# IvanTyulyandin/HMM_FASTA_Viterbi

Hardware: AMD Instinct MI355X
Metric: M residues/sec (GCUPS) for profile M=1400 vs 100k seqs, 1/2/4/8 GPU (higher is better)
Workload: dtype f32

## Files before the change

### hmm_fasta_viterbi_amd/_native.py

```python
from __future__ import annotations

import ctypes as C
import os

LIB_DIR = os.path.join(os.path.dirname(os.path.abspath(__file__)), "lib")
LIB_PATH = os.environ.get("MSV_LIB_PATH") or os.path.join(LIB_DIR, "libmsv_hip.so")

STATUS = {
    0: "MSV_OK",
    1: "MSV_ERR_INVALID_ARGUMENT",
    2: "MSV_ERR_IO",
    3: "MSV_ERR_PARSE",
    4: "MSV_ERR_BAD_RESIDUE",
    5: "MSV_ERR_SEQUENCE_TOO_LONG",
    6: "MSV_ERR_UNSUPPORTED_MODEL",
    7: "MSV_ERR_NO_DEVICE",
    8: "MSV_ERR_HIP",
    9: "MSV_ERR_OUT_OF_MEMORY",
    10: "MSV_ERR_RCCL",
}
MSV_OK = 0
MSV_ERR_BAD_RESIDUE = 4

EXPORTED = [
    "msv_status_string", "msv_version", "msv_device_count",
    "msv_hmm_read", "msv_hmm_destroy", "msv_hmm_model_length", "msv_hmm_name", "msv_hmm_stats",
    "msv_hmm_match_emissions", "msv_hmm_insert_emissions", "msv_hmm_transitions", "msv_hmm_msv_scores",
    "msv_sequence_transitions",
    "msv_fasta_read", "msv_fasta_destroy", "msv_fasta_count", "msv_fasta_rejected", "msv_fasta_codes",
    "msv_fasta_offsets", "msv_fasta_header", "msv_encode_residues",
    "msv_profile_create", "msv_profile_create_from_hmm", "msv_profile_destroy", "msv_profile_describe",
    "msv_profile_reserve_length", "msv_score_batch", "msv_score_batch_device", "msv_profile_check",
    "msv_order_longest_first", "msv_variant_count", "msv_variant_name", "msv_profile_set_variant",
    "msv_score_grid", "msv_score_grid_device", "msv_pvalues", "msv_pvalues_device",
    "msv_shard_bounds", "msv_score_batch_multi",
    "msv_fasta_parse_device", "msv_fasta_read_device", "msv_fasta_device_destroy", "msv_fasta_device_count",
    "msv_fasta_device_rejected", "msv_fasta_device_residues", "msv_fasta_device_codes", "msv_fasta_device_offsets",
    "msv_fasta_device_header_spans", "msv_fasta_device_text", "msv_fasta_device_download",
    "msv_fasta_device_max_length", "msv_score_fasta_device", "msv_fasta_device_device",
    "msv_score_batch_async", "msv_profile_wait", "msv_profile_bind_stream",
    "msv_multi_create", "msv_multi_score_batch", "msv_multi_destroy",
    "msv_host_alloc", "msv_host_free", "msv_profile_variant_for",
    "msv_filter_select_device", "msv_hmm_viterbi_scores", "msv_vit_cpu_score", "msv_vit_profile_create",
    "msv_vit_profile_create_from_hmm", "msv_vit_profile_destroy", "msv_vit_profile_reserve_length",
    "msv_vit_profile_describe", "msv_vit_variant_count", "msv_vit_variant_name", "msv_vit_profile_set_variant",
    "msv_vit_score_batch_device", "msv_vit_score_batch", "msv_vit_profile_check", "msv_vit_filter_batch",
    "msv_vit_profile_bind_stream",
    "msv_vit_cpu_trace", "msv_vit_trace_plan_count", "msv_vit_trace_plan_name", "msv_vit_trace_plan_capacity",
    "msv_vit_trace_plan_cell", "msv_vit_trace_sequence_bytes", "msv_vit_trace_chunk_cuts", "msv_vit_trace_batch",
    "msv_vit_traces_count", "msv_vit_traces_domains", "msv_vit_traces_ops", "msv_vit_traces_copy",
    "msv_vit_traces_free", "msv_vit_trace_describe", "msv_vit_traces_stats",
    "msv_fwd_cpu_score", "msv_fwd_cpu_score_batch", "msv_fwd_pvalues", "msv_fwd_scan_constants",
    "msv_fwd_profile_create", "msv_fwd_profile_create_from_hmm", "msv_fwd_profile_destroy",
    "msv_fwd_profile_reserve_length", "msv_fwd_profile_describe", "msv_fwd_variant_count", "msv_fwd_variant_name",
    "msv_fwd_profile_set_variant", "msv_fwd_score_batch_device", "msv_fwd_profile_bind_stream",
    "msv_fwd_score_batch", "msv_fwd_profile_check", "msv_fwd_pvalues_device", "msv_fwd_filter_batch",
]


class MSVError(RuntimeError):
    def __init__(self, status: int, what: str = ""):
        self.status = status
        self.name = STATUS.get(status, f"MSV_ERR_{status}")
        super().__init__(f"{what}: {self.name}" if what else self.name)


class KernelInfo(C.Structure):
    _fields_ = [
# ... 147 lines not shown
        "msv_fasta_read": (C.c_int, [C.c_char_p, C.POINTER(vp)]),
        "msv_fasta_destroy": (None, [vp]),
        "msv_fasta_count": (sz, [vp]),
        "msv_fasta_rejected": (sz, [vp]),
        "msv_fasta_codes": (C.POINTER(C.c_uint8), [vp]),
        "msv_fasta_offsets": (C.POINTER(C.c_uint64), [vp]),
        "msv_fasta_header": (C.c_char_p, [vp, sz]),
        "msv_encode_residues": (C.c_int, [C.c_char_p, sz, vp]),
        "msv_profile_create": (C.c_int, [C.c_int, vp, u32, f32, f32, f32, C.POINTER(vp)]),
        "msv_profile_create_from_hmm": (C.c_int, [C.c_int, vp, C.POINTER(vp)]),
        "msv_profile_destroy": (None, [vp]),
        "msv_profile_describe": (C.c_int, [vp, C.POINTER(KernelInfo)]),
        "msv_profile_variant_for": (C.c_char_p, [vp, C.c_uint64]),
        "msv_profile_reserve_length": (C.c_int, [vp, u64]),
        "msv_score_batch": (C.c_int, [vp, vp, vp, u64, vp, vp]),
        "msv_host_alloc": (C.c_int, [sz, C.POINTER(vp)]),
        "msv_host_free": (C.c_int, [vp]),
        "msv_score_batch_device": (C.c_int, [vp, vp, u64, vp, u64, vp, vp, vp]),
        "msv_score_batch_async": (C.c_int, [vp, vp, vp, u64, vp, C.POINTER(C.c_uint64)]),
        "msv_profile_wait": (C.c_int, [vp, u64]),
        "msv_profile_bind_stream": (C.c_int, [vp, vp]),
        "msv_multi_create": (C.c_int, [vp, C.c_uint32, C.POINTER(vp)]),
        "msv_multi_score_batch": (C.c_int, [vp, vp, vp, u64, vp]),
        "msv_multi_destroy": (None, [vp]),
        "msv_profile_check": (C.c_int, [vp, vp]),
        "msv_order_longest_first": (C.c_int, [vp, vp, u64, vp, vp]),
        "msv_variant_count": (C.c_int, []),
        "msv_variant_name": (C.c_char_p, [C.c_int]),
        "msv_profile_set_variant": (C.c_int, [vp, C.c_char_p]),
        "msv_score_grid": (C.c_int, [vp, C.c_uint32, vp, vp, u64, vp, vp]),
        "msv_score_grid_device": (C.c_int, [vp, C.c_uint32, vp, u64, vp, u64, vp, vp, vp]),
        "msv_pvalues": (C.c_int, [vp, vp, u64, C.c_float, C.c_float, vp]),
        "msv_shard_bounds": (C.c_int, [vp, u64, C.c_uint32, vp]),
        "msv_fasta_parse_device": (C.c_int, [C.c_int, vp, u64, vp, vp]),
        "msv_fasta_read_device": (C.c_int, [C.c_int, C.c_char_p, vp, vp]),
        "msv_fasta_device_destroy": (None, [vp]),
        "msv_fasta_device_count": (u64, [vp]),
        "msv_fasta_device_device": (C.c_int, [vp]),
        "msv_fasta_device_rejected": (u64, [vp]),
        "msv_fasta_device_residues": (u64, [vp]),
        "msv_fasta_device_codes": (vp, [vp]),
        "msv_fasta_device_offsets": (vp, [vp]),
        "msv_fasta_device_header_spans": (vp, [vp]),
        "msv_fasta_device_text": (vp, [vp]),
        "msv_fasta_device_download": (C.c_int, [vp, vp, vp, vp]),
        "msv_fasta_device_max_length": (u64, [vp]),
        "msv_score_fasta_device": (C.c_int, [vp, vp, vp]),
        "msv_score_batch_multi": (C.c_int, [vp, C.c_uint32, vp, vp, u64, vp]),
        "msv_pvalues_device": (C.c_int, [C.c_int, vp, vp, u64, C.c_float, C.c_float, vp, vp]),
        "msv_filter_select_device": (C.c_int, [C.c_int, vp, vp, vp, u64, f32, f32, C.c_double, vp, vp, vp, vp]),
        "msv_hmm_viterbi_scores": (C.c_int, [vp, C.c_int, vp, vp, vp, fp, fp, fp]),
        "msv_vit_cpu_score": (C.c_int, [vp, vp, vp, u32, f32, f32, f32, vp, u64, fp]),
        "msv_vit_profile_create": (C.c_int, [C.c_int, vp, vp, vp, u32, f32, f32, f32, C.POINTER(vp)]),
        "msv_vit_profile_create_from_hmm": (C.c_int, [C.c_int, vp, C.c_int, C.POINTER(vp)]),
        "msv_vit_profile_destroy": (None, [vp]),
        "msv_vit_profile_reserve_length": (C.c_int, [vp, u64]),
        "msv_vit_profile_describe": (C.c_int, [vp, C.POINTER(VitInfo)]),
        "msv_vit_variant_count": (C.c_int, []),
        "msv_vit_variant_name": (C.c_char_p, [C.c_int]),
        "msv_vit_profile_set_variant": (C.c_int, [vp, C.c_char_p]),
        "msv_vit_score_batch_device": (C.c_int, [vp, vp, u64, vp, u64, vp, vp, vp, vp]),
        "msv_vit_profile_bind_stream": (C.c_int, [vp, vp]),
        "msv_vit_score_batch": (C.c_int, [vp, vp, vp, u64, vp, vp]),
        "msv_vit_profile_check": (C.c_int, [vp, vp]),
        "msv_vit_filter_batch": (C.c_int, [vp, vp, vp, vp, u64, f32, f32, C.c_double, vp, vp, vp,
                                           C.POINTER(C.c_uint64)]),
# ... 50 lines not shown
```

### hmm_fasta_viterbi_amd/csrc/host_common.cpp

```cpp
#include <algorithm>
#include <cmath>
#include <cstdint>
#include <limits>
#include <vector>

#include "host_cpu.h"
#include "msv.h"
#include "vit_trace_plan.h"

extern "C" {

const char* msv_status_string(msv_status s) {
    switch (s) {
        case MSV_OK: return "MSV_OK";
        case MSV_ERR_INVALID_ARGUMENT: return "MSV_ERR_INVALID_ARGUMENT";
        case MSV_ERR_IO: return "MSV_ERR_IO";
        case MSV_ERR_PARSE: return "MSV_ERR_PARSE";
        case MSV_ERR_BAD_RESIDUE: return "MSV_ERR_BAD_RESIDUE";
        case MSV_ERR_SEQUENCE_TOO_LONG: return "MSV_ERR_SEQUENCE_TOO_LONG";
        case MSV_ERR_UNSUPPORTED_MODEL: return "MSV_ERR_UNSUPPORTED_MODEL";
        case MSV_ERR_NO_DEVICE: return "MSV_ERR_NO_DEVICE";
        case MSV_ERR_HIP: return "MSV_ERR_HIP";
        case MSV_ERR_OUT_OF_MEMORY: return "MSV_ERR_OUT_OF_MEMORY";
        case MSV_ERR_RCCL: return "MSV_ERR_RCCL";
// ... 79 lines not shown
    for (size_t k = 1; k + 1 < model_length; ++k)
        for (int t = 0; t < 7; ++t)
            if (!(transition_scores[k * 7 + t] <= 0.0f)) return MSV_ERR_INVALID_ARGUMENT;
    for (uint64_t i = 0; i < L; ++i)
        if (codes[i] >= 20) return MSV_ERR_BAD_RESIDUE;
    const msv_host::VitTrace t = msv_host::viterbi_trace_on_sequence(
        match_scores, insert_scores, transition_scores, model_length, tr_B_Mk, tr_E_C, tr_E_J, codes, L);
    *score = t.score;
    if (domains) {
        if (*n_domains < t.domains.size() || *n_ops < t.ops.size()) return MSV_ERR_INVALID_ARGUMENT;
        std::copy(t.domains.begin(), t.domains.end(), domains);
        std::copy(t.ops.begin(), t.ops.end(), ops);
    }
    *n_domains = static_cast<uint32_t>(t.domains.size());
    *n_ops = t.ops.size();
    return MSV_OK;
}

msv_status msv_shard_bounds(const uint64_t* offsets, uint64_t n, uint32_t n_shards, uint64_t* bounds) {
    if (!bounds || n_shards == 0 || (n && !offsets)) return MSV_ERR_INVALID_ARGUMENT;
    bounds[0] = 0;
    bounds[n_shards] = n;
    if (n == 0) {
        for (uint32_t k = 1; k < n_shards; ++k) bounds[k] = 0;
        return MSV_OK;
    }
    const uint64_t total = offsets[n] - offsets[0];
    for (uint32_t k = 1; k < n_shards; ++k) {
        const unsigned __int128 q = static_cast<unsigned __int128>(total) * k / n_shards;
        const uint64_t target = offsets[0] + static_cast<uint64_t>(q);
        bounds[k] = static_cast<uint64_t>(std::lower_bound(offsets + 1, offsets + 1 + n, target) - (offsets + 1));
    }
    for (uint32_t k = 1; k <= n_shards; ++k) bounds[k] = std::min(n, std::max(bounds[k], bounds[k - 1]));
    return MSV_OK;
}

}

namespace msv_host {

float run_on_sequence(const float* emission_scores, size_t M, float tr_B_Mk, float tr_E_C, float tr_E_J,
                      const uint8_t* codes, size_t L) {
    constexpr float ninf = -std::numeric_limits<float>::infinity();
    float loop, move;
    msv_sequence_transitions(L, &loop, &move);
    std::vector<float> prev(M, ninf), cur(M, ninf);
    float J = ninf, C = ninf, N = 0.0f, B = move;
    for (size_t i = 0; i < L; ++i) {
        const float* e = emission_scores + static_cast<size_t>(codes[i]) * M;
        const float Bt = B + tr_B_Mk;
        const float* pv = prev.data();
        float* cv = cur.data();
        for (size_t j = 1; j < M; ++j) cv[j] = e[j] + std::max(pv[j - 1], Bt);
        float Ek[8] = {ninf, ninf, ninf, ninf, ninf, ninf, ninf, ninf};
        size_t j = 1;
        for (; j + 8 <= M; j += 8)
            for (int q = 0; q < 8; ++q) Ek[q] = std::max(Ek[q], cv[j + q]);
        for (; j < M; ++j) Ek[0] = std::max(Ek[0], cv[j]);
        float E = ninf;
        for (float x : Ek) E = std::max(E, x);
        J = std::max(J + loop, E + tr_E_J);
        C = std::max(C + loop, E + tr_E_C);
        N = N + loop;
        B = std::max(N + move, J + move);
        std::swap(prev, cur);
    }
// ... 158 lines not shown
```

### hmm_fasta_viterbi_amd/csrc/host_cpu.h

```cpp
#pragma once

#include <cstddef>
#include <cstdint>
#include <vector>

#include "msv.h"

namespace msv_host {

float run_on_sequence(const float* emission_scores, size_t M, float tr_B_Mk, float tr_E_C, float tr_E_J,
                      const uint8_t* codes, size_t L);

float viterbi_run_on_sequence(const float* msc, const float* isc, const float* tsc, size_t M, float tr_B_Mk,
                              float tr_E_C, float tr_E_J, const uint8_t* codes, size_t L);

struct VitTrace {
    float score = 0;
    std::vector<msv_vit_domain> domains;
    std::vector<uint8_t> ops;
};
VitTrace viterbi_trace_on_sequence(const float* msc, const float* isc, const float* tsc, size_t M, float tr_B_Mk,
                                   float tr_E_C, float tr_E_J, const uint8_t* codes, size_t L);

std::vector<float> msv_variant_table(const float* es, uint32_t model_length, int G, int S, int sa);
std::vector<float> msv_coop_table(const float* es, uint32_t model_length, int waves, int S, int sa, int halo);
struct VitTables {
    std::vector<float> et, it, tt;
};
VitTables vit_tables(const float* msc, const float* isc_tab, const float* tsc, uint32_t model_length, int S, int team,
                     bool isc);

}
```

### hmm_fasta_viterbi_amd/csrc/msv_device.cpp

```cpp
#include <hip/hip_runtime.h>

#include <algorithm>
#include <cmath>
#include <cstdio>
#include <cstring>
#include <limits>
#include <map>
#include <memory>
#include <mutex>
#include <new>
#include <thread>
#include <vector>

#include "hip_rt.h"
#include "host_cpu.h"
#include "launch_ring.h"
#include "msv.h"
#include "msv_kernel.h"
#include "msv_plan.h"

using msvplan::CallPlan;
using msvplan::kLaunchSlots;
using msvrt::csr_extent;
using msvrt::CsrStaging;
// ... 122 lines not shown
    streams[device] = st;
    return st;
}

static bool lazy_stream(const msv_profile* p, hipStream_t st) {
    return st == p->stream || st == p->stream2 || (p->bound && st == p->bound) || (p->shared && st == p->shared);
}

static msv_status err_status(uint32_t err) {
    if (err & msvk::kErrBadOrder) return MSV_ERR_INVALID_ARGUMENT;
    if (err & msvk::kErrBadResidue) return MSV_ERR_BAD_RESIDUE;
    if (err & msvk::kErrTooLong) return MSV_ERR_SEQUENCE_TOO_LONG;
    return MSV_OK;
}

static msv_status scan_scores(const float* scores, uint64_t n) {
    bool inf = false, nan = false;
    for (uint64_t i = 0; i < n; ++i) {
        const float x = scores[i];
        inf |= x == std::numeric_limits<float>::infinity();
        nan |= x != x;
    }
    if (inf) return MSV_ERR_BAD_RESIDUE;
    if (nan) return MSV_ERR_SEQUENCE_TOO_LONG;
    return MSV_OK;
}

static msv_status grid_blocks(int device, const void* kernel, int waves, int* blocks) {
    const hipError_t e = msvrt::resident_blocks(device, kernel, waves * 64, blocks);
    return *blocks > 0 ? MSV_OK : hip_status(e);
}

static msv_status install_plan(msv_profile* p, const msvk::Variant* v, Plan& plan) {
    const std::vector<float> tab =
        msv_host::msv_variant_table(p->emission_scores.data(), p->model_length, v->G, v->S, v->sa);
    MSV_HIP(plan.d_etab.replace_with(reinterpret_cast<const float4*>(tab.data()), tab.size() / 4));
    plan.v = v;
    plan.groups_per_block = v->waves * (64 / v->G) * v->streams;
    return grid_blocks(p->device, v->fn, v->waves, &plan.blocks);
}

static void drop_plan(Plan& plan) {
    if (plan.d_etab) (void)hipDeviceSynchronize();
    plan = Plan{};
}

static msv_status install_coop_table(msv_profile* p, const msvk::CoopVariant* cv, Plan& plan) {
    const std::vector<float> tab =
        msv_host::msv_coop_table(p->emission_scores.data(), p->model_length, cv->waves, cv->S, cv->sa, cv->halo);
    MSV_HIP(plan.d_etab.replace_with(reinterpret_cast<const float4*>(tab.data()), tab.size() / 4));
    plan.v = nullptr;
    plan.cv = cv;
    plan.blocks = 0;
    plan.groups_per_block = 1;
    return MSV_OK;
}

static msv_status install_plans(msv_profile* p, int forced) {
    int cus = 0, count = 0;
    MSV_HIP(hipDeviceGetAttribute(&cus, hipDeviceAttributeMultiprocessorCount, p->device));
    const msvk::Variant* all = msvk::variants(&count);
    const msvk::CoopVariant* coop = msvk::coop_variants(&count);
    const auto blocks_of = [&](msvplan::Kind kind, int i) {
        int blocks = 0;
        if (kind == msvplan::kCoop) (void)grid_blocks(p->device, coop[i].fn, coop[i].waves, &blocks);
        else (void)grid_blocks(p->device, all[i].fn, all[i].waves, &blocks);
        return blocks;
    };
// ... 828 lines not shown
```

### hmm_fasta_viterbi_amd/csrc/msv_kernel.h

```cpp
#pragma once

#include <hip/hip_runtime.h>

#include <cstdint>

namespace msvk {

constexpr int kAminoAcids = 20;
constexpr int kPoisonRow = 20;
constexpr int kTableRows = 21;
constexpr int kWideBlocks = 64;
constexpr int kLdsLimit = 163840;

constexpr int kStampWords = 6;
constexpr int kClockTwin = -1;

constexpr uint32_t kErrBadResidue = 1u;
constexpr uint32_t kErrTooLong = 2u;
constexpr uint32_t kErrBadOrder = 4u;
constexpr uint32_t kErrTeamHang = 8u;

constexpr int lds_rows_for(int G, int S) {
    return (kLdsLimit / (G * S * 4)) >= kTableRows ? kTableRows : (kLdsLimit / (G * S * 4));
}

__device__ __host__ inline double msv_pvalue_of(float score, uint64_t L, float mu, float lambda) {
    if (L == 0) return 1.0;
    const float p1 = static_cast<float>(L) / static_cast<float>(L + 1);
    const float nullsc = static_cast<float>(static_cast<double>(L) * log(static_cast<double>(p1)) +
                                            log(1.0 - static_cast<double>(p1)));
    const float bits = (score - nullsc) / 0.69314718055994529f;
    const double y = static_cast<double>(lambda) * (static_cast<double>(bits) - static_cast<double>(mu));
    const double ey = -exp(-y);
    return fabs(ey) < 5e-9 ? -ey : 1.0 - exp(ey);
}

struct KernelArgs {
    const float4* etab;
    const uint8_t* residues;
    const uint64_t* offsets;
    const uint32_t* order;
    const float2* lentab;
    float* scores;
    uint32_t* counter;
    uint32_t* errors;
    uint64_t n;
    uint32_t lentab_n;
    float tr_B_Mk, tr_E_C, tr_E_J;
    uint64_t* stamps;
};

constexpr uint32_t kGridMaxProfiles = 32;
struct GridArgs {
    uint32_t profiles;
    uint32_t per_profile;
    KernelArgs p[kGridMaxProfiles];
// ... 39 lines not shown
```

### hmm_fasta_viterbi_amd/csrc/msv_kernel_body.inc

```
    constexpr bool SPLIT = SA > 0;
    constexpr bool WIDE = RPFO == kWideBlocks;
    constexpr bool CLOCK = RPFO == kClockTwin;
    constexpr int SW = CLOCK ? kStampWords : 4;
    constexpr int RPF0 = (RPFO > 0 && !WIDE) ? RPFO : residue_prefetch<S>();
    using St = Stream<S, (SPLIT && RPF0 < 2) ? 2 : RPF0>;
    static_assert(SPLIT ? (S - SA) % 2 == 0 : S % 4 == 0, "float4 chunks (A block), float2 halves (B block)");
    static_assert(PF >= 1 && D >= 1 && D <= 2, "PF >= 1, D in {1, 2}");
    static_assert(!SPLIT || (G >= 32 && !BIG && D == 1 && SA % 4 == 0 && SA < S), "split: 32/64-lane groups");
    constexpr int C4 = S / 4;
    constexpr int CA = SPLIT ? SA / 4 : C4;
    constexpr int HB = SPLIT ? (S - SA) / 2 : 0;
    constexpr int ROW_F4 = CA * G;
    constexpr int HBP = (HB + 1) & ~1;
    constexpr int LDS_ROWS = SPLIT ? kAminoAcids : lds_rows_for(G, S);
    constexpr bool ROT = !BIG && D == 1 && St::RPF > 1;
    constexpr int BLKN = St::RPF > 1 ? 16 : 0;
    constexpr bool BLK = !BIG && D == 1 && G >= 16 && !SPLIT && BLKN > 0;
    static_assert(!WIDE || BLK, "wide blocks are the zero-copy form of residue blocks");
    constexpr int NPH = BLK ? BLKN : St::RPF;
    constexpr bool XROW = !BIG && !SPLIT && D == 1 && PF >= C4 && St::RPF >= 2;
    constexpr bool XROW2 = XROW && NPH % 2 == 0 && PF <= 2;
    static_assert(SPLIT || BIG == (LDS_ROWS < kTableRows), "BIG <=> table does not fit LDS");
    __shared__ float4 tab[LDS_ROWS * ROW_F4];

    const float NINF = -__builtin_inff();
    const int lane = threadIdx.x & 63;
    const int gl = lane & (G - 1);
    const bool leader = gl == 0;

    for (int i = threadIdx.x; i < LDS_ROWS * ROW_F4; i += WAVES * 64) tab[i] = a.etab[i];
    __syncthreads();

    const uint8_t* __restrict__ res = a.residues;
    const float trBMk = a.tr_B_Mk, tEC = a.tr_E_C, tEJ = a.tr_E_J;
    const bool sameEJ = __float_as_uint(tEC) == __float_as_uint(tEJ);

    uint32_t rows_done = 0;
    constexpr uint32_t kFetchAhead = S >= 64 ? 8 + 256 / S : 0xFFFFFFFFu;
    constexpr uint32_t kNone = 0xFFFFFFFFu;
    const uint32_t n_groups = MSV_BLOCKS * (WAVES * 64 / G);
    static_assert(WAVES % 4 == 0, "waves are dealt in rounds of one per SIMD");
    const uint32_t wave = threadIdx.x >> 6;
    const uint32_t wave_set = a.n <= n_groups ? (wave >> 2) * 4u * MSV_BLOCKS + 4u * MSV_BLOCK + (wave & 3u)
                                              : MSV_BLOCK * WAVES + wave;
    uint32_t pending = wave_set * (64 / G) + static_cast<uint32_t>(lane / G);

    constexpr uint32_t kYoung = S >= 64 ? 8 : 0;
    const bool young = kYoung > 0 && (threadIdx.x >> 6) >= (3u * WAVES) / 4u;
    auto take = [&]() __attribute__((always_inline)) -> uint32_t {
        if constexpr (kYoung > 0) {
            if (young) {
                const uint32_t cur = group_take<G>(a.counter, false, lane, n_groups);
                if (static_cast<uint64_t>(cur) + (static_cast<uint64_t>(n_groups) * kYoung) / 4 >= a.n)
                    return 0xFFFFFFFEu;
            }
        }
        return group_take<G>(a.counter, leader, lane, n_groups);
    };
    using Ph0 = std::integral_constant<int, 0>;
    const uint32_t blk_lane = static_cast<uint32_t>(gl & (BLKN > 0 ? BLKN - 1 : 0));
    std::conditional_t<WIDE, WideBlocks, NoWideBlocks> wb;
    auto load_w = [&](uint32_t a, uint32_t e3, uint32_t& sh) __attribute__((always_inline)) -> uint32_t {
        const uint32_t a2 = min(a, e3);
        uint32_t w;
        __builtin_memcpy(&w, res + a2, 4);
        sh = (a - a2) << 3;
        return w;
    };
    const uint32_t bp_lane = WIDE ? static_cast<uint32_t>(((lane & ~15) + (blk_lane >> 2)) << 2) : 0u;
    const uint32_t bp_shift = WIDE ? (blk_lane & 3u) << 3 : 0u;
    auto extract = [&](uint32_t w, uint32_t k) __attribute__((always_inline)) -> uint32_t {
        const uint32_t v = static_cast<uint32_t>(__builtin_amdgcn_ds_bpermute(static_cast<int>(bp_lane + (k << 4)),
                                                                              static_cast<int>(w)));
        return __builtin_amdgcn_ubfe(v, bp_shift, 8);
    };

    auto begin = [&](St& st, auto ph) __attribute__((always_inline)) {
        constexpr int PH = decltype(ph)::value;
        uint32_t idx = pending;
        pending = kNone;
        if (idx == kNone) idx = take();
        const bool retire = idx >= a.n;
        uint32_t s = 0;
        uint64_t o0 = 0, o1 = 0;
        bool bad = false;
        if (!retire) {
            s = a.order ? a.order[idx] : idx;
            bad = s >= a.n;
            const uint32_t sv = bad ? 0u : s;
            o0 = a.offsets[sv];
            o1 = a.offsets[sv + 1];
        }
        const uint64_t L = o1 - o0;
        const bool empty = !retire && !bad && L == 0;
        const bool too_long = !retire && !bad && L >= a.lentab_n;
        if (leader && bad) {
            a.scores[idx] = __uint_as_float(0x7fc00000u);
            atomicOr(a.errors, kErrBadOrder);
        }
        if (leader && empty) a.scores[s] = NINF;
        if (leader && too_long) {
            a.scores[s] = __uint_as_float(0x7fc00000u);
            atomicOr(a.errors, kErrTooLong);
        }
        const bool run = !retire && !bad && !empty && !too_long;
        const float2 lm = run ? a.lentab[L] : make_float2(0.f, NINF);
        st.loop = lm.x;
        st.move = lm.y;
        st.seq = s;
        st.pos = run ? static_cast<uint32_t>(o0) : 0u;
        st.endpos = run ? static_cast<uint32_t>(o1 - 1) : 0u;
        st.endp = retire ? 0xFFFFFFFFu : (run ? static_cast<uint32_t>(o1) : 1u);
        st.ev = run ? static_cast<uint32_t>(o1 - min(L >> 1, static_cast<uint64_t>(kFetchAhead))) : st.endp;
#pragma unroll
        for (int k = 0; k < S; ++k) st.M[k] = NINF;
        st.J = NINF;
        st.C = NINF;
        st.N = 0.f;
        st.B = st.move;
        st.active = !retire;
        st.junk = !run;
        if constexpr (WIDE) {
            const uint32_t sb = st.pos - PH + 4u * blk_lane;
            wb.e3 = max(st.endpos, 3u) - 3u;
            uint32_t sh;
            wb.wcur = load_w(sb, wb.e3, sh);
            wb.wcur >>= sh;
            wb.wnext = load_w(sb + 64u, wb.e3, wb.nsh);
            wb.snext = sb + 128u;
            st.cur = min(extract(wb.wcur, 0u), static_cast<uint32_t>(kPoisonRow));
            wb.nxw = extract(wb.wcur, PH == 0 ? 0u : 1u);
            wb.wr = PH == 0 ? 1u : 2u;
        } else if constexpr (BLK) {
            const uint32_t ic = max(st.pos + blk_lane, st.pos + PH) - PH;
            const uint32_t in = PH == 0 ? ic : st.pos + blk_lane + (BLKN - PH);
            st.cur = min(static_cast<uint32_t>(res[min(ic, st.endpos)]), static_cast<uint32_t>(kPoisonRow));
            st.nxt = res[min(in, st.endpos)];
        } else {
#pragma unroll
            for (int q = 0; q < St::RPF; ++q) st.r[(PH + q) % St::RPF] = res[min(st.pos + q, st.endpos)];
        }
    };
    auto resid = [&](St& st, auto pp) __attribute__((always_inline)) -> uint32_t {
        constexpr int P = decltype(pp)::value;
        if constexpr (BLK) {
            if constexpr (P < BLKN) {
                return row_bcast_lane<P>(st.cur);
            } else {
                if constexpr (WIDE) {
                    return min(row_bcast_lane<P - BLKN>(wb.nxw), static_cast<uint32_t>(kPoisonRow));
                } else {
                    return min(row_bcast_lane<P - BLKN>(static_cast<uint32_t>(st.nxt)), static_cast<uint32_t>(kPoisonRow));
                }
            }
// ... 39 lines not shown
    };
    auto fill_ring = [&](auto& rc, const float4* ep) {
        constexpr int P = std::decay_t<decltype(rc)>::kPF;
#pragma unroll
        for (int q = 0; q < (P < CA ? P : CA); ++q) rc.ring[q] = ep[(CA - 1 - q) * G];
    };
    auto prologue = [&](St& st, auto& rc, const float4* ep, auto ph) {
        (void)ph;
        if constexpr (!BLK) rc.rnext = res[min(st.pos + St::RPF, st.endpos)];
        rc.ep = ep;
        rc.Bt = st.B + trBMk;
        if constexpr (G >= 16) {
            st.nbr = shift_in<G>(st.M[S - 1], st.nbr);
            rc.nbr = st.nbr;
        } else {
            rc.nbr = shift_in<G>(st.M[S - 1], NINF);
        }
        if constexpr (!XROW) fill_ring(rc, ep);
    };
    auto chunk = [&](St& st, auto& rc, auto cc) {
        constexpr int P = std::decay_t<decltype(rc)>::kPF;
        constexpr int c = decltype(cc)::value;
        constexpr int slot = (CA - 1 - c) % P;
        const float4 ev = rc.ring[slot];
        if constexpr (c - P >= 0) rc.ring[slot] = rc.ep[(c - P) * G];
        constexpr int k = 4 * c;
        if constexpr (!BIG && S >= 64) {
            const float mprev = c == 0 ? rc.nbr : st.M[k > 0 ? k - 1 : 0];
            asm volatile(
                "v_max_f32 %0, %1, %4\n\t"
                "v_max_f32 %1, %2, %4"
                : "+v"(st.M[k + 3]), "+v"(st.M[k + 2]), "+v"(st.M[k + 1])
                : "v"(st.M[k]), "v"(rc.Bt));
            if constexpr (!SPLIT && c == CA - 1) {
                asm volatile(
                    "v_add_f32 %0, %8, %0\n\t"
                    "v_max_f32 %2, %3, %7\n\t"
                    "v_add_f32 %1, %9, %1\n\t"
                    "v_max_f32 %3, %6, %7\n\t"
                    "v_add_f32 %2, %10, %2\n\t"
                    "v_max_f32 %4, %0, %1\n\t"
                    "v_add_f32 %3, %11, %3\n\t"
                    "v_max_f32 %5, %2, %3"
                    : "+v"(st.M[k + 3]), "+v"(st.M[k + 2]), "+v"(st.M[k + 1]), "+v"(st.M[k]), "=&v"(rc.p0),
                      "=&v"(rc.p1)
                    : "v"(mprev), "v"(rc.Bt), "v"(ev.w), "v"(ev.z), "v"(ev.y), "v"(ev.x));
            } else {
                asm volatile(
                    "v_add_f32 %0, %8, %0\n\t"
                    "v_max_f32 %2, %3, %7\n\t"
                    "v_add_f32 %1, %9, %1\n\t"
                    "v_max_f32 %3, %6, %7\n\t"
                    "v_add_f32 %2, %10, %2\n\t"
                    "v_max3_f32 %4, %4, %0, %1\n\t"
                    "v_add_f32 %3, %11, %3\n\t"
                    "v_max3_f32 %5, %5, %2, %3"
                    : "+v"(st.M[k + 3]), "+v"(st.M[k + 2]), "+v"(st.M[k + 1]), "+v"(st.M[k]), "+v"(rc.p0),
                      "+v"(rc.p1)
                    : "v"(mprev), "v"(rc.Bt), "v"(ev.w), "v"(ev.z), "v"(ev.y), "v"(ev.x));
            }
            return;
        }
        st.M[k + 3] = ev.w + fmaxf(st.M[k + 2], rc.Bt);
        st.M[k + 2] = ev.z + fmaxf(st.M[k + 1], rc.Bt);
        st.M[k + 1] = ev.y + fmaxf(st.M[k], rc.Bt);
        if constexpr (c == 0) {
            st.M[k] = ev.x + fmaxf(rc.nbr, rc.Bt);
        } else {
            st.M[k] = ev.x + fmaxf(st.M[k - 1], rc.Bt);
        }
        if constexpr (!SPLIT && c == CA - 1) {
            rc.p0 = fmaxf(st.M[k + 3], st.M[k + 2]);
            rc.p1 = fmaxf(st.M[k + 1], st.M[k]);
        } else {
            rc.p0 = fmaxf(fmaxf(rc.p0, st.M[k + 3]), st.M[k + 2]);
            rc.p1 = fmaxf(fmaxf(rc.p1, st.M[k + 1]), st.M[k]);
        }
    };
    auto bhalf = [&](St& st, auto& rc, auto hh) {
        constexpr int h = decltype(hh)::value;
        constexpr int k = SA + 2 * h;
        const float2 ev = bring.v[h];
        st.M[k + 1] = ev.y + fmaxf(st.M[k], rc.Bt);
        st.M[k] = ev.x + fmaxf(st.M[k - 1], rc.Bt);
        if constexpr (h == HB - 1) {
            rc.p0 = fmaxf(st.M[k + 1], st.M[k]);
            if constexpr (HB == 1) rc.p1 = NINF;
        } else if constexpr (h == HB - 2) {
            rc.p1 = fmaxf(st.M[k + 1], st.M[k]);
        } else if constexpr ((HB - 1 - h) & 1) {
            rc.p1 = fmaxf(fmaxf(rc.p1, st.M[k + 1]), st.M[k]);
        } else {
            rc.p0 = fmaxf(fmaxf(rc.p0, st.M[k + 1]), st.M[k]);
        }
    };
    auto epilogue = [&](St& st, auto& rc, auto ph) {
        const float Elane = fmaxf(rc.p0, rc.p1);
        const float EJ = Elane + tEJ;
        st.J = fmaxf(st.J + st.loop, EJ);
        if (__builtin_expect(!sameEJ, 0)) {
            st.C = fmaxf(st.C + st.loop, Elane + tEC);
            asm volatile("" ::: "memory");
        }
        st.N = st.N + st.loop;
        st.B = st.N + st.move;
        if (__builtin_expect(__any(st.J >= st.N), 0)) st.B = fmaxf(st.N, group_max<G>(st.J)) + st.move;
        ++st.pos;
        if constexpr (BLK) {
        } else if constexpr (ROT) {
            st.r[decltype(ph)::value] = rc.rnext;
        } else {
#pragma unroll
            for (int q = 0; q + 1 < St::RPF; ++q) st.r[q] = st.r[q + 1];
            st.r[St::RPF - 1] = rc.rnext;
        }
    };
    auto finish = [&](St& st, auto ph) __attribute__((always_inline)) {
        float csrc = st.C;
        if (sameEJ) asm volatile("v_mov_b32 %0, %1" : "=v"(csrc) : "v"(st.J));
        const float C = group_max<G>(csrc);
        const float sc = C + st.move;
        if (leader && !st.junk) {
            a.scores[st.seq] = sc;
            if (!(sc <= 3.402823466e38f)) atomicOr(a.errors, kErrBadResidue);
        }
        begin(st, ph);
    };

    St s0, s1;
    init(s0);
    if constexpr (D == 2) init(s1);

    uint64_t t_start = 0;
    uint64_t c_start = 0;
    if (a.stamps) {
        t_start = __builtin_amdgcn_s_memrealtime();
        if constexpr (CLOCK) c_start = __builtin_amdgcn_s_memtime();
    }


    RowCtx<PF> xr, xr1;
    if constexpr (XROW) fill_ring(xr, row_ptr(s0, Ph0{}));
    if constexpr (XROW2) fill_ring(xr1, lds_row(resid(s0, std::integral_constant<int, 1>{})));
    fill_b(s0.r[0]);

    auto next_slot = [](auto ph) { return (decltype(ph)::value + 1) % St::RPF; };

    auto row = [&](St& st, auto& rc, const float4* ep, auto ph) {
        prologue(st, rc, ep, ph);
        if constexpr (SPLIT) {
            [&]<int... I>(std::integer_sequence<int, I...>) {
                ((bhalf(st, rc, std::integral_constant<int, HB - 1 - I>{}),
                  [&] { if constexpr (I & 1) __builtin_amdgcn_sched_barrier(0); }()),
                 ...);
            }(std::make_integer_sequence<int, HB>{});
            fill_b(st.r[next_slot(ph)]);
            __builtin_amdgcn_sched_barrier(0);
        }
        [&]<int... I>(std::integer_sequence<int, I...>) {
            ((chunk(st, rc, std::integral_constant<int, CA - 1 - I>{}), __builtin_amdgcn_sched_barrier(0)), ...);
        }(std::make_integer_sequence<int, CA>{});
        epilogue(st, rc, ph);
    };

    bool live = __any(D == 2 ? (s0.active || s1.active) : s0.active);

    auto step = [&](auto ph) __attribute__((always_inline)) -> bool {
        constexpr int PH = decltype(ph)::value;
        constexpr int PN = (PH + 1) % NPH;
        using PhN = std::integral_constant<int, PN>;
        if constexpr (WIDE) {
            if constexpr (PH == 0) {
                s0.cur = min(wb.nxw, static_cast<uint32_t>(kPoisonRow));
                const uint32_t k = wb.wr & 3u;
                if (k == 0u) {
                    wb.wcur = wb.wnext >> wb.nsh;
                    wb.wnext = load_w(wb.snext, wb.e3, wb.nsh);
                    wb.snext += 64u;
                }
                wb.nxw = extract(wb.wcur, k);
                ++wb.wr;
            }
// ... 126 lines not shown
```

### hmm_fasta_viterbi_amd/csrc/msv_kernel_impl.h

```cpp
#pragma once
#include <hip/hip_ext.h>
#include <hip/hip_runtime.h>

#include <algorithm>
#include <cstdint>
#include <type_traits>
#include <utility>

#include "msv_kernel.h"

namespace msvk {

namespace {

template <int CTRL, int ROW_MASK = 0xF, int BANK_MASK = 0xF>
__device__ __forceinline__ float dpp(float old, float src) {
    return __int_as_float(__builtin_amdgcn_update_dpp(__float_as_int(old), __float_as_int(src), CTRL, ROW_MASK,
                                                      BANK_MASK, false));
}

constexpr int DPP_QUAD_1032 = 0xB1;
constexpr int DPP_QUAD_2301 = 0x4E;
constexpr int DPP_ROW_SHR1 = 0x111;
constexpr int DPP_ROW_MIRROR = 0x140;
// ... 54 lines not shown

template <int G>
__device__ __forceinline__ uint32_t group_take(uint32_t* counter, bool leader, int lane, uint32_t first) {
    const uint32_t v = atomicAdd(counter, leader ? 1u : 0u);
    return group_bcast<G>(v, lane) + first;
}

}

template <int S>
constexpr int residue_prefetch() {
    return S <= 16 ? 6 : (S <= 40 ? 3 : 1);
}

template <int S, int RPF_ = residue_prefetch<S>()>
struct Stream {
    static constexpr int RPF = RPF_;
    float M[S];
    float J, C, N, B, loop, move;
    float nbr;
    uint32_t pos, endpos, endp, ev, seq;
    uint8_t r[RPF];
    uint32_t cur;
    uint8_t nxt;
    bool active;
    bool junk;
};

struct WideBlocks {
    uint32_t wcur, wnext, nsh, snext, e3, wr, nxw;
};
struct NoWideBlocks {};

template <int PF>
struct RowCtx {
    static constexpr int kPF = PF;
    const float4* ep;
    float Bt, nbr, p0, p1, p2, p3;
    uint8_t rnext;
    float4 ring[PF];
};

template <int G, int S, int WAVES, int PF, bool BIG, int D, int SA = 0, int RPFO = 0>
__global__ __launch_bounds__(WAVES * 64) void msv_batch_kernel(const KernelArgs a) {
#define MSV_BLOCK blockIdx.x
#define MSV_BLOCKS gridDim.x
#include "msv_kernel_body.inc"
#undef MSV_BLOCK
#undef MSV_BLOCKS
}

template <int G, int S, int WAVES, int PF, bool BIG, int D, int SA = 0, int RPFO = 0>
__global__ __launch_bounds__(WAVES * 64) void msv_grid_kernel(const GridArgs g) {
    const uint32_t profile = blockIdx.x / g.per_profile;
    const uint32_t per_profile = g.per_profile;
    const uint32_t block_in_profile = blockIdx.x - profile * per_profile;
    const KernelArgs a = g.p[profile];
#define MSV_BLOCK block_in_profile
#define MSV_BLOCKS per_profile
#include "msv_kernel_body.inc"
#undef MSV_BLOCK
#undef MSV_BLOCKS
}

template <int G, int S, int WAVES, int PF, bool BIG, int D, int SA = 0>
constexpr const void* grid_fn() {
// ... 38 lines not shown
```

### hmm_fasta_viterbi_amd/csrc/table_layout.cpp

```cpp
#include <cstddef>
#include <cstdint>
#include <limits>
#include <vector>

#include "host_cpu.h"

namespace msv_host {

namespace {

constexpr int kAminoAcids = 20;
constexpr int kPoisonRow = 20;
constexpr int kTableRows = 21;
constexpr int kVitRows = 20;
constexpr int kVitTransitions = 7;
constexpr int kVitLanes = 64;
enum : int { MM_IN = 0, IM_IN = 1, DM_IN = 2, MI = 3, II = 4, MD_IN = 5, DD_IN = 6 };

constexpr float kNinf = -std::numeric_limits<float>::infinity();
constexpr float kPinf = std::numeric_limits<float>::infinity();

}

std::vector<float> msv_variant_table(const float* es, uint32_t model_length, int G, int S, int sa) {
    const uint32_t R = model_length - 1;
    const int C4 = S / 4;
    const float ninf = kNinf, pinf = kPinf;
    std::vector<float> tab;
    auto block = [&](int rows, int chunks, uint32_t first, int span, int width) {
        for (int r = 0; r < rows; ++r)
            for (int c = 0; c < chunks; ++c)
                for (int gl = 0; gl < G; ++gl)
                    for (int q = 0; q < width; ++q) {
                        const uint32_t j = first + static_cast<uint32_t>(gl * span + width * c + q);
                        float val;
                        if (r == kPoisonRow) val = pinf;
                        else val = (j <= R) ? es[static_cast<size_t>(r) * model_length + j] : ninf;
                        tab.push_back(val);
                    }
    };
    if (sa > 0) {
        block(kAminoAcids, sa / 4, 1, S, 4);
        const int HB = (S - sa) / 2, HBP = (HB + 1) & ~1;
        for (int r = 0; r < kTableRows; ++r)
            for (int gl = 0; gl < G; ++gl)
                for (int h = 0; h < HBP; ++h)
                    for (int q = 0; q < 2; ++q) {
                        const uint32_t j = static_cast<uint32_t>(sa + 1 + gl * S + 2 * h + q);
                        float val;
                        if (r == kPoisonRow) val = pinf;
                        else if (h < HB && j <= R) val = es[static_cast<size_t>(r) * model_length + j];
                        else val = ninf;
                        tab.push_back(val);
                    }
    } else {
        block(kTableRows, C4, 1, S, 4);
    }
    return tab;
}

std::vector<float> msv_coop_table(const float* es, uint32_t model_length, int waves, int S, int sa, int halo) {
    const uint32_t R = model_length - 1;
    const int W = waves, SA = sa, H = SA / 2, SB = S - SA;
    const float ninf = kNinf, pinf = kPinf;
    auto value = [&](int r, int w, int l, int k) {
        const int64_t j = static_cast<int64_t>(w) * (64 * S - halo) - halo + l * S + k + 1;
        if (r == kPoisonRow) return pinf;
        return (j >= 1 && j <= R) ? es[static_cast<size_t>(r) * model_length + j] : ninf;
    };
    std::vector<float> tab;
    tab.reserve(static_cast<size_t>(kTableRows) * W * 64 * S);
    for (int r = 0; r < kTableRows; ++r)
        for (int w = 0; w < W; ++w)
            for (int h = 0; h < H; ++h)
                for (int l = 0; l < 64; ++l)
                    for (int q = 0; q < 2; ++q) tab.push_back(value(r, w, l, 2 * h + q));
    for (int r = 0; r < kTableRows && SB > 0; ++r)
        for (int w = 0; w < W; ++w)
            for (int l = 0; l < 64; ++l)
                for (int i = 0; i < SB; ++i) tab.push_back(value(r, w, l, SA + i));
    return tab;
}

VitTables vit_tables(const float* msc, const float* isc_tab, const float* tsc, uint32_t model_length, int S, int team,
                     bool isc) {
    const int C2 = (S + 1) / 2, L64 = kVitLanes * team;
    const uint32_t M = model_length, K = M - 1;
    const size_t row2 = static_cast<size_t>(C2) * L64;
    auto state = [&](int l, int q) -> uint32_t { return static_cast<uint32_t>(l * S + q + 1); };
    VitTables t;
// ... 44 lines not shown
```

### include/msv.h

```cpp
#ifndef MSV_H_
#define MSV_H_

#include <stddef.h>
#include <stdint.h>

#ifdef __cplusplus
extern "C" {
#endif

typedef enum msv_status {
    MSV_OK = 0,
    MSV_ERR_INVALID_ARGUMENT = 1,
    MSV_ERR_IO = 2,
    MSV_ERR_PARSE = 3,
    MSV_ERR_BAD_RESIDUE = 4,
    MSV_ERR_SEQUENCE_TOO_LONG = 5,
    MSV_ERR_UNSUPPORTED_MODEL = 6,
    MSV_ERR_NO_DEVICE = 7,
    MSV_ERR_HIP = 8,
    MSV_ERR_OUT_OF_MEMORY = 9,
    MSV_ERR_RCCL = 10
} msv_status;

typedef struct msv_hmm msv_hmm;
// ... 82 lines not shown
msv_status msv_profile_reserve_length(msv_profile* profile, uint64_t max_length);

msv_status msv_host_alloc(size_t bytes, void** out);
msv_status msv_host_free(void* ptr);

msv_status msv_score_batch(msv_profile* profile, const uint8_t* residues, const uint64_t* offsets, uint64_t n,
                           float* scores, void* stream);

msv_status msv_score_batch_async(msv_profile* profile, const uint8_t* residues, const uint64_t* offsets, uint64_t n,
                                 float* scores, uint64_t* ticket);
msv_status msv_profile_wait(msv_profile* profile, uint64_t ticket);

msv_status msv_score_batch_device(msv_profile* profile, const uint8_t* d_residues, uint64_t residues_len,
                                  const uint64_t* d_offsets, uint64_t n, const uint32_t* d_order, float* d_scores,
                                  void* stream);

msv_status msv_profile_bind_stream(msv_profile* profile, void* stream);

msv_status msv_profile_check(msv_profile* profile, void* stream);

msv_status msv_order_longest_first(msv_profile* profile, const uint64_t* d_offsets, uint64_t n, uint32_t* d_order,
                                   void* stream);

msv_status msv_score_fasta_device(msv_profile* profile, const msv_fasta_device* fasta, float* scores);

msv_status msv_score_grid(msv_profile* const* profiles, uint32_t n_profiles, const uint8_t* residues,
                          const uint64_t* offsets, uint64_t n, float* scores, void* stream);
msv_status msv_score_grid_device(msv_profile* const* profiles, uint32_t n_profiles, const uint8_t* d_residues,
                                 uint64_t residues_len, const uint64_t* d_offsets, uint64_t n,
                                 const uint32_t* d_order, float* d_scores, void* stream);

msv_status msv_shard_bounds(const uint64_t* offsets, uint64_t n, uint32_t n_shards, uint64_t* bounds);

msv_status msv_score_batch_multi(msv_profile* const* profiles, uint32_t n_profiles, const uint8_t* residues,
                                 const uint64_t* offsets, uint64_t n, float* scores);

typedef struct msv_multi msv_multi;
msv_status msv_multi_create(msv_profile* const* profiles, uint32_t n_profiles, msv_multi** out);
msv_status msv_multi_score_batch(msv_multi* multi, const uint8_t* residues, const uint64_t* offsets, uint64_t n,
                                 float* scores);
void msv_multi_destroy(msv_multi* multi);

msv_status msv_pvalues(const float* scores, const uint64_t* offsets, uint64_t n, float mu, float lambda,
                       double* pvalues);
msv_status msv_pvalues_device(int device, const float* d_scores, const uint64_t* d_offsets, uint64_t n, float mu,
                              float lambda, double* d_pvalues, void* stream);

msv_status msv_filter_select_device(int device, const float* d_scores, const uint64_t* d_offsets,
                                    const uint32_t* d_order, uint64_t n, float mu, float lambda, double threshold,
                                    double* d_pvalues, uint32_t* d_selected, uint32_t* d_count, void* stream);

typedef struct msv_vit_profile msv_vit_profile;

typedef enum msv_insert_mode {
    MSV_INSERTS_ZERO = 0,
    MSV_INSERTS_LOG_ODDS = 1
} msv_insert_mode;

msv_status msv_hmm_viterbi_scores(const msv_hmm* hmm, int insert_mode, float* match_scores, float* insert_scores,
                                  float* transition_scores, float* tr_B_Mk, float* tr_E_C, float* tr_E_J);

msv_status msv_vit_cpu_score(const float* match_scores, const float* insert_scores, const float* transition_scores,
                             uint32_t model_length, float tr_B_Mk, float tr_E_C, float tr_E_J, const uint8_t* codes,
                             uint64_t L, float* score);

msv_status msv_vit_profile_create(int device, const float* match_scores, const float* insert_scores,
// ... 153 lines not shown
```

Measured before the change: 13400.

## Add lazy E-state evaluation using per-lane emission upper bounds

For the non-big, single-stream, S>=68 variant, the kernel keeps a per-lane upper bound U on match scores, built from a new per-residue, per-lane max-emission table stored in LDS after the main table. The full per-row E reduction and J update run only when the bound could beat the group's current J; otherwise that work is skipped. The per-row E max that was folded into the match asm is removed and replaced by a bound update plus a wave-wide compare, with group_max called only when needed. This costs extra LDS, a few ALU ops and a ballot per row, and is only correct if the bound logic is conservative.

```diff
diff --git a/hmm_fasta_viterbi_amd/_native.py b/hmm_fasta_viterbi_amd/_native.py
--- a/hmm_fasta_viterbi_amd/_native.py
+++ b/hmm_fasta_viterbi_amd/_native.py
@@ -33,7 +33,7 @@
     "msv_profile_reserve_length", "msv_score_batch", "msv_score_batch_device", "msv_profile_check",
     "msv_order_longest_first", "msv_variant_count", "msv_variant_name", "msv_profile_set_variant",
     "msv_score_grid", "msv_score_grid_device", "msv_pvalues", "msv_pvalues_device",
-    "msv_shard_bounds", "msv_score_batch_multi",
+    "msv_shard_bounds", "msv_lazy_bound_table", "msv_score_batch_multi",
     "msv_fasta_parse_device", "msv_fasta_read_device", "msv_fasta_device_destroy", "msv_fasta_device_count",
     "msv_fasta_device_rejected", "msv_fasta_device_residues", "msv_fasta_device_codes", "msv_fasta_device_offsets",
     "msv_fasta_device_header_spans", "msv_fasta_device_text", "msv_fasta_device_download",
@@ -247,6 +247,7 @@
         "msv_score_grid_device": (C.c_int, [vp, C.c_uint32, vp, u64, vp, u64, vp, vp, vp]),
         "msv_pvalues": (C.c_int, [vp, vp, u64, C.c_float, C.c_float, vp]),
         "msv_shard_bounds": (C.c_int, [vp, u64, C.c_uint32, vp]),
+        "msv_lazy_bound_table": (C.c_int, [vp, C.c_uint32, C.c_int, C.c_int, vp]),
         "msv_fasta_parse_device": (C.c_int, [C.c_int, vp, u64, vp, vp]),
         "msv_fasta_read_device": (C.c_int, [C.c_int, C.c_char_p, vp, vp]),
         "msv_fasta_device_destroy": (None, [vp]),
diff --git a/hmm_fasta_viterbi_amd/csrc/host_common.cpp b/hmm_fasta_viterbi_amd/csrc/host_common.cpp
--- a/hmm_fasta_viterbi_amd/csrc/host_common.cpp
+++ b/hmm_fasta_viterbi_amd/csrc/host_common.cpp
@@ -135,6 +135,13 @@
         bounds[k] = static_cast<uint64_t>(std::lower_bound(offsets + 1, offsets + 1 + n, target) - (offsets + 1));
     }
     for (uint32_t k = 1; k <= n_shards; ++k) bounds[k] = std::min(n, std::max(bounds[k], bounds[k - 1]));
+    return MSV_OK;
+}
+
+msv_status msv_lazy_bound_table(const float* emission_scores, uint32_t model_length, int G, int S, float* out) {
+    if (!emission_scores || !out || model_length < 2 || G <= 0 || S <= 0) return MSV_ERR_INVALID_ARGUMENT;
+    const std::vector<float> tab = msv_host::msv_lazy_bound_table(emission_scores, model_length, G, S);
+    std::copy(tab.begin(), tab.end(), out);
     return MSV_OK;
 }
 
diff --git a/hmm_fasta_viterbi_amd/csrc/host_cpu.h b/hmm_fasta_viterbi_amd/csrc/host_cpu.h
--- a/hmm_fasta_viterbi_amd/csrc/host_cpu.h
+++ b/hmm_fasta_viterbi_amd/csrc/host_cpu.h
@@ -23,6 +23,7 @@
                                    float tr_E_C, float tr_E_J, const uint8_t* codes, size_t L);
 
 std::vector<float> msv_variant_table(const float* es, uint32_t model_length, int G, int S, int sa);
+std::vector<float> msv_lazy_bound_table(const float* es, uint32_t model_length, int G, int S);
 std::vector<float> msv_coop_table(const float* es, uint32_t model_length, int waves, int S, int sa, int halo);
 struct VitTables {
     std::vector<float> et, it, tt;
diff --git a/hmm_fasta_viterbi_amd/csrc/msv_device.cpp b/hmm_fasta_viterbi_amd/csrc/msv_device.cpp
--- a/hmm_fasta_viterbi_amd/csrc/msv_device.cpp
+++ b/hmm_fasta_viterbi_amd/csrc/msv_device.cpp
@@ -178,8 +178,13 @@
 }
 
 static msv_status install_plan(msv_profile* p, const msvk::Variant* v, Plan& plan) {
-    const std::vector<float> tab =
+    std::vector<float> tab =
         msv_host::msv_variant_table(p->emission_scores.data(), p->model_length, v->G, v->S, v->sa);
+    if (msvk::lazy_e_rows(v->S, v->waves, v->pf, v->big, v->sa, v->streams)) {
+        const std::vector<float> emax =
+            msv_host::msv_lazy_bound_table(p->emission_scores.data(), p->model_length, v->G, v->S);
+        tab.insert(tab.end(), emax.begin(), emax.end());
+    }
     MSV_HIP(plan.d_etab.replace_with(reinterpret_cast<const float4*>(tab.data()), tab.size() / 4));
     plan.v = v;
     plan.groups_per_block = v->waves * (64 / v->G) * v->streams;
diff --git a/hmm_fasta_viterbi_amd/csrc/msv_kernel.h b/hmm_fasta_viterbi_amd/csrc/msv_kernel.h
--- a/hmm_fasta_viterbi_amd/csrc/msv_kernel.h
+++ b/hmm_fasta_viterbi_amd/csrc/msv_kernel.h
@@ -22,6 +22,10 @@
 
 constexpr int lds_rows_for(int G, int S) {
     return (kLdsLimit / (G * S * 4)) >= kTableRows ? kTableRows : (kLdsLimit / (G * S * 4));
+}
+
+constexpr bool lazy_e_rows(int S, int waves, int pf, bool big, int sa, int streams) {
+    return !big && sa == 0 && streams == 1 && S >= 68 && waves == 16 && pf == 2;
 }
 
 __device__ __host__ inline double msv_pvalue_of(float score, uint64_t L, float mu, float lambda) {
diff --git a/hmm_fasta_viterbi_amd/csrc/msv_kernel_body.inc b/hmm_fasta_viterbi_amd/csrc/msv_kernel_body.inc
--- a/hmm_fasta_viterbi_amd/csrc/msv_kernel_body.inc
+++ b/hmm_fasta_viterbi_amd/csrc/msv_kernel_body.inc
@@ -21,14 +21,17 @@
     constexpr bool XROW = !BIG && !SPLIT && D == 1 && PF >= C4 && St::RPF >= 2;
     constexpr bool XROW2 = XROW && NPH % 2 == 0 && PF <= 2;
     static_assert(SPLIT || BIG == (LDS_ROWS < kTableRows), "BIG <=> table does not fit LDS");
-    __shared__ float4 tab[LDS_ROWS * ROW_F4];
+    constexpr bool LAZY = lazy_e_rows(S, WAVES, PF, BIG, SA, D);
+    constexpr int EMAX_F4 = LAZY ? kTableRows * G / 4 : 0;
+    static_assert((LDS_ROWS * ROW_F4 + EMAX_F4) * 16 <= kLdsLimit, "table and bound table fit LDS");
+    __shared__ float4 tab[LDS_ROWS * ROW_F4 + EMAX_F4];
 
     const float NINF = -__builtin_inff();
     const int lane = threadIdx.x & 63;
     const int gl = lane & (G - 1);
     const bool leader = gl == 0;
 
-    for (int i = threadIdx.x; i < LDS_ROWS * ROW_F4; i += WAVES * 64) tab[i] = a.etab[i];
+    for (int i = threadIdx.x; i < LDS_ROWS * ROW_F4 + EMAX_F4; i += WAVES * 64) tab[i] = a.etab[i];
     __syncthreads();
 
     const uint8_t* __restrict__ res = a.residues;
@@ -60,6 +63,7 @@
     using Ph0 = std::integral_constant<int, 0>;
     const uint32_t blk_lane = static_cast<uint32_t>(gl & (BLKN > 0 ? BLKN - 1 : 0));
     std::conditional_t<WIDE, WideBlocks, NoWideBlocks> wb;
+    std::conditional_t<LAZY, LazyE, NoLazyE> lz;
     auto load_w = [&](uint32_t a, uint32_t e3, uint32_t& sh) __attribute__((always_inline)) -> uint32_t {
         const uint32_t a2 = min(a, e3);
         uint32_t w;
@@ -120,6 +124,10 @@
         st.B = st.move;
         st.active = !retire;
         st.junk = !run;
+        if constexpr (LAZY) {
+            lz.U = NINF;
+            lz.Jg = NINF;
+        }
         if constexpr (WIDE) {
             const uint32_t sb = st.pos - PH + 4u * blk_lane;
             wb.e3 = max(st.endpos, 3u) - 3u;
@@ -225,7 +233,17 @@
                 "v_max_f32 %1, %2, %4"
                 : "+v"(st.M[k + 3]), "+v"(st.M[k + 2]), "+v"(st.M[k + 1])
                 : "v"(st.M[k]), "v"(rc.Bt));
-            if constexpr (!SPLIT && c == CA - 1) {
+            if constexpr (LAZY) {
+                asm volatile(
+                    "v_add_f32 %0, %6, %0\n\t"
+                    "v_max_f32 %2, %3, %5\n\t"
+                    "v_add_f32 %1, %7, %1\n\t"
+                    "v_max_f32 %3, %4, %5\n\t"
+                    "v_add_f32 %2, %8, %2\n\t"
+                    "v_add_f32 %3, %9, %3"
+                    : "+v"(st.M[k + 3]), "+v"(st.M[k + 2]), "+v"(st.M[k + 1]), "+v"(st.M[k])
+                    : "v"(mprev), "v"(rc.Bt), "v"(ev.w), "v"(ev.z), "v"(ev.y), "v"(ev.x));
+            } else if constexpr (!SPLIT && c == CA - 1) {
                 asm volatile(
                     "v_add_f32 %0, %8, %0\n\t"
                     "v_max_f32 %2, %3, %7\n\t"
@@ -288,12 +306,31 @@
         }
     };
     auto epilogue = [&](St& st, auto& rc, auto ph) {
-        const float Elane = fmaxf(rc.p0, rc.p1);
-        const float EJ = Elane + tEJ;
-        st.J = fmaxf(st.J + st.loop, EJ);
-        if (__builtin_expect(!sameEJ, 0)) {
-            st.C = fmaxf(st.C + st.loop, Elane + tEC);
-            asm volatile("" ::: "memory");
+        if constexpr (LAZY) {
+            float Jn = st.J + st.loop;
+            if (lz.full != 0) {
+                float e4[4] = {st.M[0], st.M[1], st.M[2], st.M[3]};
+#pragma unroll
+                for (int q = 4; q + 1 < S; q += 2) e4[(q / 2) & 3] = fmaxf(fmaxf(e4[(q / 2) & 3], st.M[q]), st.M[q + 1]);
+                const float Elane = fmaxf(fmaxf(e4[0], e4[1]), fmaxf(e4[2], e4[3]));
+                const float EJ = Elane + tEJ;
+                Jn = fmaxf(Jn, EJ);
+                lz.U = Elane;
+                if (__builtin_expect(__any(EJ > lz.Jg), 0)) lz.Jg = group_max<G>(Jn);
+                if (__builtin_expect(!sameEJ, 0)) {
+                    st.C = fmaxf(st.C + st.loop, Elane + tEC);
+                    asm volatile("" ::: "memory");
+                }
+            }
+            st.J = Jn;
+        } else {
+            const float Elane = fmaxf(rc.p0, rc.p1);
+            const float EJ = Elane + tEJ;
+            st.J = fmaxf(st.J + st.loop, EJ);
+            if (__builtin_expect(!sameEJ, 0)) {
+                st.C = fmaxf(st.C + st.loop, Elane + tEC);
+                asm volatile("" ::: "memory");
+            }
         }
         st.N = st.N + st.loop;
         st.B = st.N + st.move;
@@ -339,8 +376,20 @@
 
     auto next_slot = [](auto ph) { return (decltype(ph)::value + 1) % St::RPF; };
 
+    const uint64_t lazy_off = sameEJ ? 0ull : ~0ull;
     auto row = [&](St& st, auto& rc, const float4* ep, auto ph) {
+        float lazy_em = 0.f;
+        if constexpr (LAZY) {
+            const uint32_t r = resid(st, ph);
+            const uint32_t rr = BLK ? r : min(r, static_cast<uint32_t>(kPoisonRow));
+            lazy_em = reinterpret_cast<const float*>(tab + LDS_ROWS * ROW_F4)[rr * G + static_cast<uint32_t>(gl)];
+        }
         prologue(st, rc, ep, ph);
+        if constexpr (LAZY) {
+            lz.U = lazy_em + fmaxf(fmaxf(lz.U, rc.nbr), rc.Bt);
+            lz.Jg = lz.Jg + st.loop;
+            lz.full = __builtin_amdgcn_fcmpf(lz.U + tEJ, lz.Jg, 2 ) | lazy_off;
+        }
         if constexpr (SPLIT) {
             [&]<int... I>(std::integer_sequence<int, I...>) {
                 ((bhalf(st, rc, std::integral_constant<int, HB - 1 - I>{}),
diff --git a/hmm_fasta_viterbi_amd/csrc/msv_kernel_impl.h b/hmm_fasta_viterbi_amd/csrc/msv_kernel_impl.h
--- a/hmm_fasta_viterbi_amd/csrc/msv_kernel_impl.h
+++ b/hmm_fasta_viterbi_amd/csrc/msv_kernel_impl.h
@@ -110,6 +110,12 @@
 };
 struct NoWideBlocks {};
 
+struct LazyE {
+    float U, Jg;
+    uint64_t full;
+};
+struct NoLazyE {};
+
 template <int PF>
 struct RowCtx {
     static constexpr int kPF = PF;
diff --git a/hmm_fasta_viterbi_amd/csrc/table_layout.cpp b/hmm_fasta_viterbi_amd/csrc/table_layout.cpp
--- a/hmm_fasta_viterbi_amd/csrc/table_layout.cpp
+++ b/hmm_fasta_viterbi_amd/csrc/table_layout.cpp
@@ -56,6 +56,22 @@
     } else {
         block(kTableRows, C4, 1, S, 4);
     }
+    return tab;
+}
+
+std::vector<float> msv_lazy_bound_table(const float* es, uint32_t model_length, int G, int S) {
+    const uint32_t R = model_length - 1;
+    std::vector<float> tab(static_cast<size_t>(kTableRows) * G, kPinf);
+    for (int r = 0; r < kAminoAcids; ++r)
+        for (int gl = 0; gl < G; ++gl) {
+            float m = kNinf;
+            for (int q = 0; q < S; ++q) {
+                const uint32_t j = 1 + static_cast<uint32_t>(gl * S + q);
+                if (j <= R && es[static_cast<size_t>(r) * model_length + j] > m)
+                    m = es[static_cast<size_t>(r) * model_length + j];
+            }
+            tab[static_cast<size_t>(r) * G + gl] = m;
+        }
     return tab;
 }
 
diff --git a/include/msv.h b/include/msv.h
--- a/include/msv.h
+++ b/include/msv.h
@@ -138,6 +138,8 @@
 
 msv_status msv_shard_bounds(const uint64_t* offsets, uint64_t n, uint32_t n_shards, uint64_t* bounds);
 
+msv_status msv_lazy_bound_table(const float* emission_scores, uint32_t model_length, int G, int S, float* out);
+
 msv_status msv_score_batch_multi(msv_profile* const* profiles, uint32_t n_profiles, const uint8_t* residues,
                                  const uint64_t* offsets, uint64_t n, float* scores);
 
```

After: 13770, median of 6. 1.03x the previous value.
